# glmanhtu/vit-ed

Measured on AMD Instinct MI355X. Metric: patch-pairs/sec fwd+bwd, div2k_erosion7_4bin_patch8_64 ViT-ED, higher is better.
Workload: dtype bf16

## Files before the change

### vit-ed_amd/csrc/context_fold.hip

```cpp
#include "common.h"

#define CF_MAX_BLOCKS 16

struct FoldArgs {
    const float* w[CF_MAX_BLOCKS];
    const float* bias[CF_MAX_BLOCKS];
    const float* gamma[CF_MAX_BLOCKS];
    const float* beta[CF_MAX_BLOCKS];
    bf16* w_out;
    bf16* wt_out;
    float* bias_out;
    int count, N, K;
};

__global__ void __launch_bounds__(256) fold_context_kernel(const FoldArgs a) {
    const int lane = threadIdx.x & 63;
    const int row = blockIdx.x * 4 + (threadIdx.x >> 6);
    if (row >= a.count * a.N) return;
    const int l = row / a.N, n = row - l * a.N;
    const float* __restrict__ w = a.w[l] + (int64_t)n * a.K;
    const float* __restrict__ g = a.gamma[l];
    const float* __restrict__ be = a.beta[l];
    const int64_t ldt = (int64_t)a.count * a.N;
    float dot = 0.f;
    for (int k = lane; k < a.K; k += 64) {
        const float wv = w[k];
        const bf16 f = (bf16)(wv * g[k]);
        a.w_out[(int64_t)row * a.K + k] = f;
        a.wt_out[(int64_t)k * ldt + row] = f;
        dot = fmaf(wv, be[k], dot);
    }
    dot = wave_sum(dot);
    if (lane == 0) a.bias_out[row] = dot + (a.bias[l] ? a.bias[l][n] : 0.f);
}

extern "C" int vited_fold_context_weights(int count, const float* const* w, const float* const* bias, const float* const* gamma,
                                          const float* const* beta, int64_t N, int64_t K, void* w_out, void* wt_out, float* bias_out,
                                          void* stream) {
    if (count < 1 || count > CF_MAX_BLOCKS || !w || !bias || !gamma || !beta || !w_out || !wt_out || !bias_out || N <= 0 || K <= 0)
        return VITED_ERR_BAD_ARG;
    FoldArgs a = {};
    for (int i = 0; i < count; ++i) {
        if (!w[i] || !gamma[i] || !beta[i]) return VITED_ERR_BAD_ARG;
        a.w[i] = w[i]; a.bias[i] = bias[i]; a.gamma[i] = gamma[i]; a.beta[i] = beta[i];
    }
    a.w_out = (bf16*)w_out; a.wt_out = (bf16*)wt_out; a.bias_out = bias_out;
    a.count = count; a.N = (int)N; a.K = (int)K;
    hipLaunchKernelGGL(fold_context_kernel, dim3((unsigned)ceil_div64((int64_t)count * N, 4)), dim3(256), 0, (hipStream_t)stream, a);
    return vited_check_launch();
}

struct UnfoldArgs {
    const float* w[CF_MAX_BLOCKS];
    const float* gamma[CF_MAX_BLOCKS];
    const float* beta[CF_MAX_BLOCKS];
    float* dw[CF_MAX_BLOCKS];
    float* dbias[CF_MAX_BLOCKS];
    float* dgamma[CF_MAX_BLOCKS];
    float* dbeta[CF_MAX_BLOCKS];
    const float* dwf;
    const float* dbf;
    int count, N, K, accumulate;
};

#define UF_GROUPS 16
__global__ void __launch_bounds__(64 * UF_GROUPS) unfold_context_kernel(const UnfoldArgs a) {
    __shared__ float red[2][UF_GROUPS][64];
    const int l = blockIdx.y, kx = threadIdx.x & 63, ng = threadIdx.x >> 6;
    const int k = blockIdx.x * 64 + kx;
    const bool ok = k < a.K;
    const float* __restrict__ w = a.w[l];
    const float* __restrict__ dwf = a.dwf + (int64_t)l * a.N * a.K;
    const float* __restrict__ dbf = a.dbf + (int64_t)l * a.N;
    float* __restrict__ dw = a.dw[l];
    const float g = ok ? a.gamma[l][k] : 0.f, be = ok ? a.beta[l][k] : 0.f;
    float sg = 0.f, sb = 0.f;
#pragma unroll 4
    for (int n = ng; n < a.N; n += UF_GROUPS) {
        if (ok) {
            const int64_t o = (int64_t)n * a.K + k;
            const float d = dwf[o], wv = w[o], dbn = dbf[n];
            sg = fmaf(d, wv, sg);
            sb = fmaf(dbn, wv, sb);
            const float v = fmaf(d, g, dbn * be);
            dw[o] = a.accumulate ? dw[o] + v : v;
        }
    }
    red[0][ng][kx] = sg;
    red[1][ng][kx] = sb;
    __syncthreads();
    if (ng == 0 && ok) {
        float tg = 0.f, tb = 0.f;
#pragma unroll
        for (int w = 0; w < UF_GROUPS; ++w) {
            tg += red[0][w][kx];
            tb += red[1][w][kx];
        }
        a.dgamma[l][k] = a.accumulate ? a.dgamma[l][k] + tg : tg;
        a.dbeta[l][k] = a.accumulate ? a.dbeta[l][k] + tb : tb;
    }
    if (blockIdx.x == 0 && a.dbias[l]) {
        for (int n = threadIdx.x; n < a.N; n += 64 * UF_GROUPS) a.dbias[l][n] = a.accumulate ? a.dbias[l][n] + dbf[n] : dbf[n];
    }
}

extern "C" int vited_unfold_context_grads(int count, const float* dwf, const float* dbf, const float* const* w, const float* const* gamma,
                                          const float* const* beta, float* const* dw, float* const* dbias, float* const* dgamma, float* const* dbeta, int64_t N,
                                          int64_t K, int accumulate, void* stream) {
    if (count < 1 || count > CF_MAX_BLOCKS || !dwf || !dbf || !w || !gamma || !beta || !dw || !dbias || !dgamma || !dbeta || N <= 0 || K <= 0)
        return VITED_ERR_BAD_ARG;
    UnfoldArgs a = {};
    for (int i = 0; i < count; ++i) {
        if (!w[i] || !gamma[i] || !beta[i] || !dw[i] || !dgamma[i] || !dbeta[i]) return VITED_ERR_BAD_ARG;
        a.w[i] = w[i]; a.gamma[i] = gamma[i]; a.beta[i] = beta[i]; a.dw[i] = dw[i]; a.dbias[i] = dbias[i]; a.dgamma[i] = dgamma[i]; a.dbeta[i] = dbeta[i];
    }
    a.dwf = dwf; a.dbf = dbf; a.count = count; a.N = (int)N; a.K = (int)K; a.accumulate = accumulate;
    hipLaunchKernelGGL(unfold_context_kernel, dim3((unsigned)ceil_div64(K, 64), (unsigned)count), dim3(64 * UF_GROUPS), 0, (hipStream_t)stream, a);
    return vited_check_launch();
}
```

### vit-ed_amd/csrc/elementwise.hip

```cpp
#include "common.h"

template <typename S, typename D>
__global__ void cast_kernel(const S* __restrict__ src, D* __restrict__ dst, int64_t n) {
    int64_t i = ((int64_t)blockIdx.x * blockDim.x + threadIdx.x) * 4;
    const int64_t stride = (int64_t)gridDim.x * blockDim.x * 4;
    for (; i + 3 < n; i += stride) {
        S a = src[i], b = src[i + 1], c = src[i + 2], d = src[i + 3];
        dst[i] = from_f32<D>(to_f32(a));
        dst[i + 1] = from_f32<D>(to_f32(b));
        dst[i + 2] = from_f32<D>(to_f32(c));
        dst[i + 3] = from_f32<D>(to_f32(d));
    }
    for (; i < n; ++i) dst[i] = from_f32<D>(to_f32(src[i]));
}

extern "C" int vited_cast(const void* src, int src_dtype, void* dst, int dst_dtype, int64_t n, void* stream) {
    if (!src || !dst || n < 0) return VITED_ERR_BAD_ARG;
    if (n == 0) return VITED_OK;
    hipStream_t s = (hipStream_t)stream;
    const int threads = 256;
    int64_t blocks = ceil_div64(n, threads * 4);
    if (blocks > 4096) blocks = 4096;
    if (src_dtype == VITED_F32 && dst_dtype == VITED_BF16)
        hipLaunchKernelGGL((cast_kernel<float, bf16>), dim3(blocks), dim3(threads), 0, s, (const float*)src, (bf16*)dst, n);
    else if (src_dtype == VITED_BF16 && dst_dtype == VITED_F32)
        hipLaunchKernelGGL((cast_kernel<bf16, float>), dim3(blocks), dim3(threads), 0, s, (const bf16*)src, (float*)dst, n);
    else if (src_dtype == VITED_F32 && dst_dtype == VITED_F32)
        hipLaunchKernelGGL((cast_kernel<float, float>), dim3(blocks), dim3(threads), 0, s, (const float*)src, (float*)dst, n);
    else if (src_dtype == VITED_BF16 && dst_dtype == VITED_BF16)
        hipLaunchKernelGGL((cast_kernel<bf16, bf16>), dim3(blocks), dim3(threads), 0, s, (const bf16*)src, (bf16*)dst, n);
    else
        return VITED_ERR_UNSUPPORTED;
    return vited_check_launch();
}

template <typename D>
__global__ void __launch_bounds__(256)
scale_rows_cast_kernel(const float* __restrict__ src, int64_t src_ld, const float* __restrict__ scale, D* __restrict__ dst, int64_t dst_ld,
                       int64_t rows, int dim) {
    const int hl = threadIdx.x & 31;
    const int64_t half = ((int64_t)blockIdx.x * blockDim.x + threadIdx.x) >> 5;
    const int64_t nhalf = ((int64_t)gridDim.x * blockDim.x) >> 5;
    for (int64_t r = half; r < rows; r += nhalf) {
        const float sc = scale[r];
        for (int c = hl * 4; c < dim; c += 128) {
            const f32x4 v = *(const f32x4*)(src + r * src_ld + c);
            if constexpr (sizeof(D) == 2) {
                *(bf16x4*)((bf16*)dst + r * dst_ld + c) = bf16x4{(bf16)(sc * v[0]), (bf16)(sc * v[1]), (bf16)(sc * v[2]), (bf16)(sc * v[3])};
            } else {
                *(f32x4*)((float*)dst + r * dst_ld + c) = f32x4{sc * v[0], sc * v[1], sc * v[2], sc * v[3]};
            }
        }
    }
}

extern "C" int vited_scale_rows_cast(const float* src, int64_t src_ld, const float* row_scale, void* dst, int dst_dtype, int64_t dst_ld,
                                     int64_t rows, int64_t dim, void* stream) {
    if (!src || !row_scale || !dst || rows <= 0 || dim <= 0 || src_ld < dim || dst_ld < dim) return VITED_ERR_BAD_ARG;
    if (dim % 4 || src_ld % 4 || dst_ld % 4 || dim > (1 << 20)) return VITED_ERR_UNSUPPORTED;
    if (((uintptr_t)src & 15) || ((uintptr_t)dst & (dst_dtype == VITED_F32 ? 15 : 7))) return VITED_ERR_BAD_ARG;
    int64_t blocks = ceil_div64(rows, 8);
    if (blocks > 2048) blocks = 2048;
    hipStream_t s = (hipStream_t)stream;
    if (dst_dtype == VITED_BF16)
        hipLaunchKernelGGL((scale_rows_cast_kernel<bf16>), dim3(blocks), dim3(256), 0, s, src, src_ld, row_scale, (bf16*)dst, dst_ld, rows, (int)dim);
    else if (dst_dtype == VITED_F32)
        hipLaunchKernelGGL((scale_rows_cast_kernel<float>), dim3(blocks), dim3(256), 0, s, src, src_ld, row_scale, (float*)dst, dst_ld, rows, (int)dim);
    else
        return VITED_ERR_UNSUPPORTED;
    return vited_check_launch();
}

template <typename D>
__global__ void cast_transpose_kernel(const float* __restrict__ src, D* __restrict__ dst, int64_t rows, int64_t cols) {
    __shared__ float tile[32][33];
    const int64_t c0 = (int64_t)blockIdx.x * 32, r0 = (int64_t)blockIdx.y * 32;
    const int tx = threadIdx.x & 31, ty = threadIdx.x >> 5;
    for (int j = ty; j < 32; j += 8) {
        int64_t r = r0 + j, c = c0 + tx;
        tile[j][tx] = (r < rows && c < cols) ? src[r * cols + c] : 0.f;
    }
    __syncthreads();
    for (int j = ty; j < 32; j += 8) {
        int64_t c = c0 + j, r = r0 + tx;
        if (c < cols && r < rows) dst[c * rows + r] = from_f32<D>(tile[tx][j]);
    }
}

extern "C" int vited_cast_transpose(const float* src, void* dst, int dst_dtype, int64_t rows, int64_t cols, void* stream) {
    if (!src || !dst || rows <= 0 || cols <= 0) return VITED_ERR_BAD_ARG;
    dim3 grid((unsigned)ceil_div64(cols, 32), (unsigned)ceil_div64(rows, 32));
    hipStream_t s = (hipStream_t)stream;
    if (dst_dtype == VITED_BF16)
        hipLaunchKernelGGL((cast_transpose_kernel<bf16>), grid, dim3(256), 0, s, src, (bf16*)dst, rows, cols);
    else if (dst_dtype == VITED_F32)
        hipLaunchKernelGGL((cast_transpose_kernel<float>), grid, dim3(256), 0, s, src, (float*)dst, rows, cols);
    else
        return VITED_ERR_UNSUPPORTED;
    return vited_check_launch();
}

#define WS_DESC_WORDS 6
__global__ void __launch_bounds__(256)
cast_weights_kernel(const int64_t* __restrict__ desc, int count) {
    __shared__ bf16 tile[64][66];
    const int64_t blk = blockIdx.x;
    int lo = 0, hi = count - 1;
    while (lo < hi) {
        const int mid = (lo + hi + 1) >> 1;
        if (desc[(int64_t)mid * WS_DESC_WORDS + 5] <= blk) lo = mid; else hi = mid - 1;
    }
    const int64_t* d = desc + (int64_t)lo * WS_DESC_WORDS;
    const float* __restrict__ src = (const float*)d[0];
    bf16* __restrict__ dst = (bf16*)d[1];
    bf16* __restrict__ dst_t = (bf16*)d[2];
    const int64_t rows = d[3], cols = d[4];
    const int64_t t = blk - d[5], tiles_c = (cols + 63) >> 6;
    const int64_t r0 = (t / tiles_c) << 6, c0 = (t % tiles_c) << 6;
    const int tx = threadIdx.x & 15, ty = threadIdx.x >> 4;
    const bool vec = (cols & 3) == 0;
#pragma unroll
    for (int j = 0; j < 4; ++j) {
        const int lr = ty + 16 * j;
        const int64_t r = r0 + lr, c = c0 + tx * 4;
        float v[4] = {0.f, 0.f, 0.f, 0.f};
        if (r < rows) {
            if (vec && c + 3 < cols) {
                const f32x4 q = *(const f32x4*)(src + r * cols + c);
                v[0] = q[0]; v[1] = q[1]; v[2] = q[2]; v[3] = q[3];
            } else {
#pragma unroll
                for (int e = 0; e < 4; ++e) if (c + e < cols) v[e] = src[r * cols + c + e];
            }
        }
        bf16 b[4];
#pragma unroll
        for (int e = 0; e < 4; ++e) { b[e] = (bf16)v[e]; tile[lr][tx * 4 + e] = b[e]; }
        if (dst && r < rows) {
            if (vec && c + 3 < cols) *(bf16x4*)(dst + r * cols + c) = bf16x4{b[0], b[1], b[2], b[3]};
            else {
#pragma unroll
                for (int e = 0; e < 4; ++e) if (c + e < cols) dst[r * cols + c + e] = b[e];
            }
        }
    }
    if (!dst_t) return;
    __syncthreads();
    const bool vec_t = (rows & 3) == 0;
#pragma unroll
    for (int j = 0; j < 4; ++j) {
        const int lc = ty + 16 * j;
        const int64_t c = c0 + lc, r = r0 + tx * 4;
        if (c >= cols) continue;
        bf16 b[4];
#pragma unroll
        for (int e = 0; e < 4; ++e) b[e] = tile[tx * 4 + e][lc];
        if (vec_t && r + 3 < rows) *(bf16x4*)(dst_t + c * rows + r) = bf16x4{b[0], b[1], b[2], b[3]};
        else {
#pragma unroll
            for (int e = 0; e < 4; ++e) if (r + e < rows) dst_t[c * rows + r + e] = b[e];
        }
    }
}

extern "C" int vited_cast_weights(const int64_t* desc, int count, int64_t total_tiles, void* stream) {
    if (!desc || count <= 0 || total_tiles <= 0 || total_tiles > 0x7fffffff) return VITED_ERR_BAD_ARG;
    hipLaunchKernelGGL(cast_weights_kernel, dim3((unsigned)total_tiles), dim3(256), 0, (hipStream_t)stream, desc, count);
    return vited_check_launch();
}

template <typename D>
__global__ void patchify_kernel(const float* __restrict__ img, int64_t img_bs, const int64_t* __restrict__ bidx,
                                D* __restrict__ out, int chans, int S, int p) {
    const int G = S / p;
    const int64_t b = blockIdx.y;
    const int py = blockIdx.x;
    const int64_t src_b = bidx ? bidx[b] : b;
    const float* base = img + src_b * img_bs;
    const int Kp = chans * p * p;
    const int total = chans * p * S;
    D* obase = out + (b * G * G + (int64_t)py * G) * Kp;
    for (int e = threadIdx.x; e < total; e += blockDim.x) {
        const int x = e % S;
        const int ci = e / S;
        const int i = ci % p, c = ci / p;
        const float v = base[((int64_t)c * S + (py * p + i)) * S + x];
        const int px = x / p, j = x - px * p;
        obase[(int64_t)px * Kp + (c * p + i) * p + j] = from_f32<D>(v);
    }
}

extern "C" int vited_patchify(const float* img, int64_t img_bs, const int64_t* batch_index, void* out, int out_dtype,
                              int64_t batch, int chans, int img_size, int patch, void* stream) {
    if (!img || !out || batch <= 0 || chans <= 0 || img_size <= 0 || patch <= 0 || img_size % patch) return VITED_ERR_BAD_ARG;
    dim3 grid(img_size / patch, (unsigned)batch);
    hipStream_t s = (hipStream_t)stream;
    if (out_dtype == VITED_BF16)
        hipLaunchKernelGGL((patchify_kernel<bf16>), grid, dim3(256), 0, s, img, img_bs, batch_index, (bf16*)out, chans, img_size, patch);
    else if (out_dtype == VITED_F32)
        hipLaunchKernelGGL((patchify_kernel<float>), grid, dim3(256), 0, s, img, img_bs, batch_index, (float*)out, chans, img_size, patch);
    else
        return VITED_ERR_UNSUPPORTED;
    return vited_check_launch();
}

struct U8Norm { float scale[4], shift[4]; };

template <typename D>
__global__ void patchify_u8_kernel(const uint8_t* __restrict__ img, int64_t img_bs, const int64_t* __restrict__ bidx,
                                   D* __restrict__ out, int chans, int S, int p, U8Norm nrm) {
    const int G = S / p;
    const int64_t b = blockIdx.y;
    const int py = blockIdx.x;
    const int64_t src_b = bidx ? bidx[b] : b;
    const uint8_t* base = img + src_b * img_bs;
    const int Kp = chans * p * p;
    const int total = chans * p * S;
    D* obase = out + (b * G * G + (int64_t)py * G) * Kp;
    for (int e = threadIdx.x; e < total; e += blockDim.x) {
        const int x = e % S;
        const int ci = e / S;
        const int i = ci % p, c = ci / p;
        const float v = fmaf((float)base[((int64_t)c * S + (py * p + i)) * S + x], nrm.scale[c], nrm.shift[c]);
        const int px = x / p, j = x - px * p;
        obase[(int64_t)px * Kp + (c * p + i) * p + j] = from_f32<D>(v);
    }
}

extern "C" int vited_patchify_u8(const uint8_t* img, int64_t img_bs, const int64_t* batch_index, void* out, int out_dtype,
                                 int64_t batch, int chans, int img_size, int patch, const float* mean, const float* std,
                                 void* stream) {
    if (!img || !out || !mean || !std || batch <= 0 || chans <= 0 || chans > 4 || img_size <= 0 || patch <= 0 || img_size % patch)
        return VITED_ERR_BAD_ARG;
    U8Norm nrm = {};
    for (int c = 0; c < chans; ++c) {
        if (!(std[c] > 0.f)) return VITED_ERR_BAD_ARG;
        nrm.scale[c] = 1.0f / (255.0f * std[c]);
        nrm.shift[c] = -mean[c] / std[c];
    }
    dim3 grid(img_size / patch, (unsigned)batch);
    hipStream_t s = (hipStream_t)stream;
    if (out_dtype == VITED_BF16)
        hipLaunchKernelGGL((patchify_u8_kernel<bf16>), grid, dim3(256), 0, s, img, img_bs, batch_index, (bf16*)out, chans, img_size, patch, nrm);
    else if (out_dtype == VITED_F32)
        hipLaunchKernelGGL((patchify_u8_kernel<float>), grid, dim3(256), 0, s, img, img_bs, batch_index, (float*)out, chans, img_size, patch, nrm);
    else
        return VITED_ERR_UNSUPPORTED;
    return vited_check_launch();
}

struct ResampleTaps {
    int x0, n;
    int k0, k1;
};

__device__ __forceinline__ ResampleTaps resample_taps(int xx, int in_size, int out_size) {
    constexpr int PRECISION_BITS = 32 - 8 - 2;
    const double scale = (double)in_size / (double)out_size;
    const double center = (xx + 0.5) * scale;
    int xmin = (int)(center - 1.0 + 0.5);
    xmin = xmin < 0 ? 0 : xmin;
    int xmax = (int)(center + 1.0 + 0.5);
    xmax = (xmax < in_size ? xmax : in_size) - xmin;
    double w0 = 1.0 - fabs((double)xmin - center + 0.5), w1 = xmax > 1 ? 1.0 - fabs((double)xmin + 1.0 - center + 0.5) : 0.0;
    w0 = w0 < 0.0 ? 0.0 : w0;
    w1 = w1 < 0.0 ? 0.0 : w1;
    const double ww = w0 + w1;
    ResampleTaps t;
    t.x0 = xmin;
    t.n = xmax > 1 ? 2 : 1;
    t.k0 = (int)(0.5 + (w0 / ww) * (double)(1 << PRECISION_BITS));
    t.k1 = (int)(0.5 + (w1 / ww) * (double)(1 << PRECISION_BITS));
    return t;
}

__device__ __forceinline__ int resample_px(int p0, int p1, const ResampleTaps& t) {
    constexpr int PRECISION_BITS = 32 - 8 - 2;
    int acc = (1 << (PRECISION_BITS - 1)) + p0 * t.k0 + (t.n > 1 ? p1 * t.k1 : 0);
    acc >>= PRECISION_BITS;
    return acc < 0 ? 0 : (acc > 255 ? 255 : acc);
}

__global__ void __launch_bounds__(256)
crop_pairs_u8_kernel(const uint8_t* __restrict__ src, int64_t src_bs, const int* __restrict__ cells, const int* __restrict__ erode,
                     uint8_t* __restrict__ out, int chans, int S) {
    const int64_t b = blockIdx.z;
    const int img = blockIdx.y / chans, c = blockIdx.y % chans;
    int cell = cells[b * 2 + img], e = erode[b];
    cell = cell < 0 ? 0 : (cell > 5 ? 5 : cell);
    e = e < 1 ? 1 : (e > S ? S : e);
    const int off = (int)rint((S - e) / 2.0);
    const int r0 = (cell / 3) * S + off, c0 = (cell % 3) * S + off;
    const uint8_t* base = src + b * src_bs + ((int64_t)c * 2 * S + r0) * (3 * S) + c0;
    uint8_t* o = out + (((b * 2 + img) * chans + c) * (int64_t)S) * S;
    for (int i = blockIdx.x * blockDim.x + threadIdx.x; i < S * S; i += gridDim.x * blockDim.x) {
        const int y = i / S, x = i - y * S;
        const ResampleTaps tx = resample_taps(x, e, S), ty = resample_taps(y, e, S);
        const uint8_t* ra = base + (int64_t)ty.x0 * (3 * S) + tx.x0;
        const int h0 = resample_px(ra[0], tx.n > 1 ? ra[1] : 0, tx);
        int h1 = 0;
        if (ty.n > 1) {
            const uint8_t* rb = ra + 3 * S;
            h1 = resample_px(rb[0], tx.n > 1 ? rb[1] : 0, tx);
        }
        o[i] = (uint8_t)resample_px(h0, h1, ty);
    }
}

extern "C" int vited_crop_pairs_u8(const uint8_t* src, int64_t src_bs, const int* cells, const int* erode, uint8_t* out, int64_t batch,
                                   int chans, int img_size, void* stream) {
    if (!src || !cells || !erode || !out || batch <= 0 || chans <= 0 || img_size <= 0 || batch > 65535) return VITED_ERR_BAD_ARG;
    if (src_bs < (int64_t)chans * 6 * img_size * img_size) return VITED_ERR_BAD_ARG;
    const int per = img_size * img_size;
    dim3 grid((unsigned)((per + 1023) / 1024 < 8 ? (per + 1023) / 1024 : 8), (unsigned)(2 * chans), (unsigned)batch);
    hipLaunchKernelGGL(crop_pairs_u8_kernel, grid, dim3(256), 0, (hipStream_t)stream, src, src_bs, cells, erode, out, chans, img_size);
    return vited_check_launch();
}

template <typename D>
__global__ void slice_rows_cast_kernel(const float* __restrict__ in, D* __restrict__ out, int64_t in_rows,
                                       int64_t row_offset, int64_t rows, int64_t dim, int64_t total) {
    int64_t i = (int64_t)blockIdx.x * blockDim.x + threadIdx.x;
    const int64_t stride = (int64_t)gridDim.x * blockDim.x;
    const int64_t per_b = rows * dim;
    for (; i < total; i += stride) {
        const int64_t b = i / per_b, rem = i - b * per_b;
        out[i] = from_f32<D>(in[(b * in_rows + row_offset) * dim + rem]);
    }
}

extern "C" int vited_slice_rows_cast(const float* in, void* out, int out_dtype, int64_t batch, int64_t in_rows,
                                     int64_t row_offset, int64_t rows, int64_t dim, void* stream) {
    if (!in || !out || batch <= 0 || rows <= 0 || dim <= 0 || row_offset < 0 || row_offset + rows > in_rows) return VITED_ERR_BAD_ARG;
    const int64_t total = batch * rows * dim;
    int64_t blocks = ceil_div64(total, 256);
    if (blocks > 8192) blocks = 8192;
    hipStream_t s = (hipStream_t)stream;
    if (out_dtype == VITED_BF16)
        hipLaunchKernelGGL((slice_rows_cast_kernel<bf16>), dim3(blocks), dim3(256), 0, s, in, (bf16*)out, in_rows, row_offset, rows, dim, total);
    else if (out_dtype == VITED_F32)
        hipLaunchKernelGGL((slice_rows_cast_kernel<float>), dim3(blocks), dim3(256), 0, s, in, (float*)out, in_rows, row_offset, rows, dim, total);
    else
        return VITED_ERR_UNSUPPORTED;
    return vited_check_launch();
}

__global__ void write_cls_row_kernel(float* __restrict__ x, const float* __restrict__ cls, const float* __restrict__ pos,
                                     int64_t batch, int64_t rows_per_batch, int64_t dim) {
    int64_t i = (int64_t)blockIdx.x * blockDim.x + threadIdx.x;
    const int64_t total = batch * dim;
    if (i >= total) return;
    const int64_t b = i / dim, d = i - b * dim;
    x[b * rows_per_batch * dim + d] = cls[d] + pos[d];
}

extern "C" int vited_write_cls_row(float* x, const float* cls, const float* pos, int64_t batch, int64_t rows_per_batch,
                                   int64_t dim, void* stream) {
    if (!x || !cls || !pos || batch <= 0 || rows_per_batch <= 0 || dim <= 0) return VITED_ERR_BAD_ARG;
    const int64_t total = batch * dim;
    hipLaunchKernelGGL(write_cls_row_kernel, dim3((unsigned)ceil_div64(total, 256)), dim3(256), 0, (hipStream_t)stream,
                       x, cls, pos, batch, rows_per_batch, dim);
    return vited_check_launch();
}

template <typename S_>
__global__ void sum_rows_kernel(const S_* __restrict__ in, int64_t in_ld, float* __restrict__ out, int64_t batch,
                                int64_t width, int64_t rows_per_split) {
    const int64_t r = (int64_t)blockIdx.x * blockDim.x + threadIdx.x;
    if (r >= width) return;
    const int64_t b0 = (int64_t)blockIdx.y * rows_per_split;
    int64_t b1 = b0 + rows_per_split;
    if (b1 > batch) b1 = batch;
    float acc0 = 0.f, acc1 = 0.f, acc2 = 0.f, acc3 = 0.f;
    int64_t b = b0;
    for (; b + 3 < b1; b += 4) {
        acc0 += to_f32(in[b * in_ld + r]);
        acc1 += to_f32(in[(b + 1) * in_ld + r]);
        acc2 += to_f32(in[(b + 2) * in_ld + r]);
        acc3 += to_f32(in[(b + 3) * in_ld + r]);
    }
    for (; b < b1; ++b) acc0 += to_f32(in[b * in_ld + r]);
    out[(int64_t)blockIdx.y * width + r] = (acc0 + acc1) + (acc2 + acc3);
}

static inline int64_t sum_rows_splits(int64_t batch, int64_t width) {
    const int64_t col_blocks = ceil_div64(width, 256);
    int64_t s = ceil_div64(1024, col_blocks);
    const int64_t max_s = ceil_div64(batch, 16);
    if (s > max_s) s = max_s;
    if (s < 1) s = 1;
    return s;
}

extern "C" int64_t vited_sum_rows_workspace_bytes(int64_t batch, int64_t width) {
    return sum_rows_splits(batch, width) * width * (int64_t)sizeof(float);
// ... 165 lines not shown
```

### vit-ed_amd/csrc/patch_keep.hip

```cpp
#include "common.h"
#include "patch_keep.h"

__global__ void __launch_bounds__(256)
keep_from_keys_kernel(const float* __restrict__ keys, int* __restrict__ keep, int L, int K) {
    __shared__ float row[PK_MAX_KEYS];
    const int64_t b = blockIdx.x;
    const float* src = keys + b * L;
    for (int i = threadIdx.x; i < L; i += blockDim.x) row[i] = src[i];
    __syncthreads();
    for (int i = threadIdx.x; i < L; i += blockDim.x) {
        const int rank = pk_rank(row, L, i);
        if (rank < K) keep[b * K + rank] = i;
    }
}

extern "C" int vited_keep_from_keys(const float* keys, int32_t* keep, int64_t batch, int L, int K, void* stream) {
    if (!keys || !keep || batch <= 0 || batch > 0x7fffffff || L <= 0 || K <= 0 || K > L) return VITED_ERR_BAD_ARG;
    if (((uintptr_t)keys | (uintptr_t)keep) % 4) return VITED_ERR_BAD_ARG;
    if (L > PK_MAX_KEYS) return VITED_ERR_UNSUPPORTED;
    hipLaunchKernelGGL(keep_from_keys_kernel, dim3((unsigned)batch), dim3(256), 0, (hipStream_t)stream, keys, keep, L, K);
    return vited_check_launch();
}

struct PkNorm { float scale[4], shift[4]; };

template <typename S, typename D>
__global__ void __launch_bounds__(256)
patchify_kept_kernel(const S* __restrict__ img, int64_t img_bs, const int64_t* __restrict__ bidx, const int* __restrict__ keep, int K,
                     int lead, D* __restrict__ out, int chans, int img_size, int p, PkNorm nrm) {
    const int G = img_size / p, R = pk_rows(K, lead);
    const int64_t b = blockIdx.x;
    const int r = blockIdx.y;
    const int patch = pk_patch(keep + b * K, lead, r, G * G);
    const int py = patch / G, px = patch - py * G;
    const int64_t src_b = bidx ? bidx[b] : b;
    const S* base = img + src_b * img_bs + (int64_t)(py * p) * img_size + px * p;
    const int Kp = chans * p * p;
    D* o = out + (b * R + r) * (int64_t)Kp;
    for (int e = threadIdx.x; e < Kp; e += blockDim.x) {
        const int j = e % p, ci = e / p;
        const int i = ci % p, c = ci / p;
        const S raw = base[((int64_t)c * img_size + i) * img_size + j];
        float v;
        if constexpr (sizeof(S) == 1) v = fmaf((float)raw, nrm.scale[c], nrm.shift[c]);
        else v = raw;
        o[e] = from_f32<D>(v);
    }
}

static int patchify_kept_args(const void* img, const int32_t* keep, int K, int lead, const void* out, int64_t batch, int chans,
                              int img_size, int patch) {
    if (!img || !keep || !out || batch <= 0 || batch > 0x7fffffff || chans <= 0 || img_size <= 0 || patch <= 0 || img_size % patch)
        return VITED_ERR_BAD_ARG;
    const int64_t n = (int64_t)(img_size / patch) * (img_size / patch);
    if ((lead != 0 && lead != 1) || K <= 0 || (int64_t)K + lead > n || (uintptr_t)keep % 4) return VITED_ERR_BAD_ARG;
    if (pk_rows(K, lead) > 65535) return VITED_ERR_UNSUPPORTED;
    return VITED_OK;
}

extern "C" int vited_patchify_kept(const float* img, int64_t img_bs, const int64_t* batch_index, const int32_t* keep, int K, int lead,
                                   void* out, int out_dtype, int64_t batch, int chans, int img_size, int patch, void* stream) {
    if (int err = patchify_kept_args(img, keep, K, lead, out, batch, chans, img_size, patch)) return err;
    if ((uintptr_t)img % 4) return VITED_ERR_BAD_ARG;
    dim3 grid((unsigned)batch, (unsigned)pk_rows(K, lead));
    hipStream_t s = (hipStream_t)stream;
    const PkNorm none = {};
    if (out_dtype == VITED_BF16)
        hipLaunchKernelGGL((patchify_kept_kernel<float, bf16>), grid, dim3(256), 0, s, img, img_bs, batch_index, keep, K, lead, (bf16*)out,
                           chans, img_size, patch, none);
    else if (out_dtype == VITED_F32)
        hipLaunchKernelGGL((patchify_kept_kernel<float, float>), grid, dim3(256), 0, s, img, img_bs, batch_index, keep, K, lead, (float*)out,
                           chans, img_size, patch, none);
    else
        return VITED_ERR_UNSUPPORTED;
    return vited_check_launch();
}

extern "C" int vited_patchify_kept_u8(const uint8_t* img, int64_t img_bs, const int64_t* batch_index, const int32_t* keep, int K, int lead,
                                      void* out, int out_dtype, int64_t batch, int chans, int img_size, int patch, const float* mean,
                                      const float* std, void* stream) {
    if (int err = patchify_kept_args(img, keep, K, lead, out, batch, chans, img_size, patch)) return err;
    if (!mean || !std || chans > 4) return VITED_ERR_BAD_ARG;
    PkNorm nrm = {};
    for (int c = 0; c < chans; ++c) {
        if (!(std[c] > 0.f)) return VITED_ERR_BAD_ARG;
        nrm.scale[c] = 1.0f / (255.0f * std[c]);
        nrm.shift[c] = -mean[c] / std[c];
    }
    dim3 grid((unsigned)batch, (unsigned)pk_rows(K, lead));
    hipStream_t s = (hipStream_t)stream;
    if (out_dtype == VITED_BF16)
        hipLaunchKernelGGL((patchify_kept_kernel<uint8_t, bf16>), grid, dim3(256), 0, s, img, img_bs, batch_index, keep, K, lead, (bf16*)out,
                           chans, img_size, patch, nrm);
    else if (out_dtype == VITED_F32)
        hipLaunchKernelGGL((patchify_kept_kernel<uint8_t, float>), grid, dim3(256), 0, s, img, img_bs, batch_index, keep, K, lead,
                           (float*)out, chans, img_size, patch, nrm);
    else
        return VITED_ERR_UNSUPPORTED;
    return vited_check_launch();
}

__global__ void __launch_bounds__(256)
tokens_kept_kernel(const float* __restrict__ tok, const float* __restrict__ pos, const float* __restrict__ cls, const int* __restrict__ keep,
                   int K, int lead, float* __restrict__ x, int64_t total, int n_patches, int dim4) {
    const int R = pk_rows(K, lead), first = cls ? 1 : 0, rows = R + first;
    const int64_t stride = (int64_t)gridDim.x * blockDim.x;
    for (int64_t i = (int64_t)blockIdx.x * blockDim.x + threadIdx.x; i < total; i += stride) {
        const int64_t row = i / dim4;
        const int c = (int)(i - row * dim4) * 4;
        const int64_t b = row / rows;
        const int t = (int)(row - b * rows);
        f32x4 v;
        if (t < first) {
            v = *(const f32x4*)(cls + c) + *(const f32x4*)(pos + c);
        } else {
            const int r = t - first;
            const int patch = pk_patch(keep + b * K, lead, r, n_patches);
            v = *(const f32x4*)(tok + (b * R + r) * (int64_t)(dim4 * 4) + c) + *(const f32x4*)(pos + (int64_t)(1 + patch) * (dim4 * 4) + c);
        }
        *(f32x4*)(x + row * (int64_t)(dim4 * 4) + c) = v;
    }
}

extern "C" int vited_tokens_kept(const float* tok, const float* pos, const float* cls, const int32_t* keep, int K, int lead, float* x,
                                 int64_t batch, int n_patches, int dim, void* stream) {
    if (!tok || !pos || !keep || !x || batch <= 0 || n_patches <= 0 || dim <= 0 || dim % 4) return VITED_ERR_BAD_ARG;
    if ((lead != 0 && lead != 1) || K <= 0 || (int64_t)K + lead > n_patches || (uintptr_t)keep % 4) return VITED_ERR_BAD_ARG;
    if (((uintptr_t)tok | (uintptr_t)pos | (uintptr_t)cls | (uintptr_t)x) % 16) return VITED_ERR_BAD_ARG;
    const int64_t total = batch * (pk_rows(K, lead) + (cls ? 1 : 0)) * (dim / 4);
    int64_t blocks = ceil_div64(total, 256);
    if (blocks > 8192) blocks = 8192;
    hipLaunchKernelGGL(tokens_kept_kernel, dim3((unsigned)blocks), dim3(256), 0, (hipStream_t)stream, tok, pos, cls, keep, K, lead, x, total,
                       n_patches, dim / 4);
    return vited_check_launch();
}

__global__ void __launch_bounds__(256)
keep_inverse_kernel(const int* __restrict__ keep, int K, int lead, int* __restrict__ inv, int n_patches) {
    const int64_t b = blockIdx.x;
    int* mine = inv + b * n_patches;
    pk_inverse_clear(mine, n_patches, threadIdx.x, blockDim.x);
    __syncthreads();
    pk_inverse_fill(mine, keep + b * K, K, lead, n_patches, threadIdx.x, blockDim.x);
}

extern "C" int vited_keep_inverse(const int32_t* keep, int K, int lead, int32_t* inv, int64_t batch, int n_patches, void* stream) {
    if (!keep || !inv || batch <= 0 || batch > 0x7fffffff || n_patches <= 0) return VITED_ERR_BAD_ARG;
    if ((lead != 0 && lead != 1) || K <= 0 || (int64_t)K + lead > n_patches || ((uintptr_t)keep | (uintptr_t)inv) % 4) return VITED_ERR_BAD_ARG;
    hipLaunchKernelGGL(keep_inverse_kernel, dim3((unsigned)batch), dim3(256), 0, (hipStream_t)stream, keep, K, lead, inv, n_patches);
    return vited_check_launch();
}

__global__ void __launch_bounds__(256)
tokens_kept_bwd_kernel(const float* __restrict__ dx, const int* __restrict__ inv, float* __restrict__ dpos, float* __restrict__ dcls,
                       int64_t batch, int rows, int first, int n_patches, int dim4) {
    const int64_t i = (int64_t)blockIdx.x * blockDim.x + threadIdx.x;
    if (i >= (int64_t)(n_patches + 1) * dim4) return;
    const int q = (int)(i / dim4), c = (int)(i - (int64_t)q * dim4) * 4;
    const int dim = dim4 * 4, R = rows - first;
    f32x4 acc = {0.f, 0.f, 0.f, 0.f};
    if (q == 0) {
        if (first)
            for (int64_t b = 0; b < batch; ++b) acc += *(const f32x4*)(dx + b * rows * (int64_t)dim + c);
        if (dcls) *(f32x4*)(dcls + c) = acc;
    } else {
        const int* col = inv + (q - 1);
        int64_t b = 0;
        for (; b + 4 <= batch; b += 4) {
            int r[4];
#pragma unroll
            for (int u = 0; u < 4; ++u) r[u] = col[(b + u) * n_patches];
            f32x4 v[4];
#pragma unroll
            for (int u = 0; u < 4; ++u) {
                const bool kept = r[u] >= 0 && r[u] < R;
                v[u] = kept ? *(const f32x4*)(dx + ((b + u) * rows + first + (kept ? r[u] : 0)) * (int64_t)dim + c) : f32x4{0.f, 0.f, 0.f, 0.f};
            }
#pragma unroll
            for (int u = 0; u < 4; ++u)
                if (r[u] >= 0 && r[u] < R) acc += v[u];
        }
        for (; b < batch; ++b) {
            const int r = col[b * n_patches];
            if (r >= 0 && r < R) acc += *(const f32x4*)(dx + (b * rows + first + r) * (int64_t)dim + c);
        }
    }
    *(f32x4*)(dpos + (int64_t)q * dim + c) = acc;
}

extern "C" int vited_tokens_kept_bwd(const float* dx, const int32_t* inv, float* dpos, float* dcls, int64_t batch, int rows, int with_cls,
                                     int n_patches, int dim, void* stream) {
    if (!dx || !inv || !dpos || batch <= 0 || n_patches <= 0 || dim <= 0 || dim % 4 || (with_cls != 0 && with_cls != 1)) return VITED_ERR_BAD_ARG;
    if (rows <= with_cls || rows - with_cls > n_patches || (!with_cls && dcls)) return VITED_ERR_BAD_ARG;
    if (((uintptr_t)dx | (uintptr_t)dpos | (uintptr_t)dcls) % 16 || (uintptr_t)inv % 4) return VITED_ERR_BAD_ARG;
    const int64_t total = (int64_t)(n_patches + 1) * (dim / 4);
    hipLaunchKernelGGL(tokens_kept_bwd_kernel, dim3((unsigned)ceil_div64(total, 256)), dim3(256), 0, (hipStream_t)stream, dx, inv, dpos,
                       dcls, batch, rows, with_cls, n_patches, dim / 4);
    return vited_check_launch();
}
```

Baseline: 43860.

## Tile context fold transpose, deepen unfold loads, vectorise patchify row runs

The context-weight fold kernel now processes 32 rows per block and stages results in shared memory, so the transposed bf16 output is written as coalesced 4-wide vectors instead of strided scalar stores. The unfold gradient kernel is templated on column width and accumulate mode, batches many loads ahead of use for memory-level parallelism, and picks a narrower width when the grid would be small. The patchify and kept-patchify paths gain kernels where each thread moves one contiguous patch row with vector loads and stores, falling back to the old kernels when alignment fails. A profiling helper script is added. Register pressure from the deeper unrolling and extra template instances are the main risks.

Measured after the change: 43890, median of 3. No clear change (+0.1%).

```diff
diff --git a/profiles/step_kernels.py b/profiles/step_kernels.py
--- /dev/null
+++ b/profiles/step_kernels.py
@@ -0,0 +1,53 @@
+#!/usr/bin/env python3
+import collections
+import csv
+import glob
+import os
+import statistics
+import sys
+
+
+def main():
+    args = [a for a in sys.argv[1:] if not a.startswith('--')]
+    src, dst = args[0], args[1]
+    window = None
+    if '--window' in sys.argv:
+        window = int(sys.argv[sys.argv.index('--window') + 1])
+    trace = max(glob.glob(os.path.join(src, '**', '*_kernel_trace.csv'), recursive=True), key=os.path.getmtime)
+    rows = []
+    for r in csv.DictReader(open(trace)):
+        rows.append((int(r['Start_Timestamp']), int(r['End_Timestamp']), r['Kernel_Name']))
+    rows.sort()
+    os.makedirs(dst, exist_ok=True)
+
+    per = collections.defaultdict(list)
+    for s, e, n in rows:
+        per[n].append(e - s)
+    with open(os.path.join(dst, 'kernel_stats.csv'), 'w') as f:
+        f.write('Name,Calls,TotalDurationNs,AverageNs,MedianNs\n')
+        for n, d in sorted(per.items(), key=lambda kv: -sum(kv[1]))[:60]:
+            f.write(f'"{n[:110]}",{len(d)},{sum(d)},{sum(d) // len(d)},{int(statistics.median(d))}\n')
+
+    ends = [i for i, (_, _, n) in enumerate(rows) if 'optim_update_kernel' in n or 'adamw_update_kernel' in n]
+    first_u8 = next((i for i, (_, _, n) in enumerate(rows) if 'patchify_u8' in n or 'patchify_run_kernelIh' in n
+                     or 'patchify_run_kernel<unsigned char' in n), len(rows))
+    wins = [(ends[k - 1] + 1, ends[k] + 1) for k in range(1, len(ends))]
+    for k, (a, b) in enumerate(wins):
+        print(f'window {k}: {b - a} kernels, wall {(rows[b - 1][1] - rows[a][0]) / 1e6:.3f} ms, '
+              f'busy {sum(e - s for s, e, _ in rows[a:b]) / 1e6:.3f} ms')
+    if window is None:
+        window = max(k for k, (a, b) in enumerate(wins) if b <= first_u8)
+    a, b = wins[window]
+    print(f'chosen window {window}')
+    step = collections.defaultdict(list)
+    for s, e, n in rows[a:b]:
+        step[n].append(e - s)
+    with open(os.path.join(dst, 'step_kernels.csv'), 'w') as f:
+        f.write('Name,Launches,TotalUs,AverageUs\n')
+        for n, d in sorted(step.items(), key=lambda kv: -sum(kv[1])):
+            f.write(f'"{n[:110]}",{len(d)},{sum(d) / 1e3:.2f},{sum(d) / len(d) / 1e3:.2f}\n')
+    print(f'step: {b - a} kernels, wall {(rows[b - 1][1] - rows[a][0]) / 1e6:.3f} ms, busy {sum(e - s for s, e, _ in rows[a:b]) / 1e6:.3f} ms')
+
+
+if __name__ == '__main__':
+    main()
diff --git a/vit-ed_amd/csrc/context_fold.hip b/vit-ed_amd/csrc/context_fold.hip
--- a/vit-ed_amd/csrc/context_fold.hip
+++ b/vit-ed_amd/csrc/context_fold.hip
@@ -13,25 +13,72 @@
     int count, N, K;
 };
 
+#define FC_ROWS 32
+#define FC_PER_WAVE (FC_ROWS / 4)
 __global__ void __launch_bounds__(256) fold_context_kernel(const FoldArgs a) {
-    const int lane = threadIdx.x & 63;
-    const int row = blockIdx.x * 4 + (threadIdx.x >> 6);
-    if (row >= a.count * a.N) return;
-    const int l = row / a.N, n = row - l * a.N;
-    const float* __restrict__ w = a.w[l] + (int64_t)n * a.K;
-    const float* __restrict__ g = a.gamma[l];
-    const float* __restrict__ be = a.beta[l];
-    const int64_t ldt = (int64_t)a.count * a.N;
-    float dot = 0.f;
-    for (int k = lane; k < a.K; k += 64) {
-        const float wv = w[k];
-        const bf16 f = (bf16)(wv * g[k]);
-        a.w_out[(int64_t)row * a.K + k] = f;
-        a.wt_out[(int64_t)k * ldt + row] = f;
-        dot = fmaf(wv, be[k], dot);
+    __shared__ bf16 tile[64][FC_ROWS + 4];
+    const int lane = threadIdx.x & 63, wave = threadIdx.x >> 6;
+    const int rows = a.count * a.N;
+    const int row0 = blockIdx.x * FC_ROWS;
+    const int64_t ldt = rows;
+    const bool vec_t = (ldt & 3) == 0 && ((uintptr_t)a.wt_out & 7) == 0;
+    const float* w[FC_PER_WAVE];
+    const float* g[FC_PER_WAVE];
+    const float* be[FC_PER_WAVE];
+    float dot[FC_PER_WAVE];
+#pragma unroll
+    for (int j = 0; j < FC_PER_WAVE; ++j) {
+        const int row = row0 + wave * FC_PER_WAVE + j;
+        const int l = row < rows ? row / a.N : 0, n = row < rows ? row - l * a.N : 0;
+        w[j] = a.w[l] + (int64_t)n * a.K;
+        g[j] = a.gamma[l];
+        be[j] = a.beta[l];
+        dot[j] = 0.f;
     }
-    dot = wave_sum(dot);
-    if (lane == 0) a.bias_out[row] = dot + (a.bias[l] ? a.bias[l][n] : 0.f);
+    for (int k0 = 0; k0 < a.K; k0 += 64) {
+        const int k = k0 + lane;
+        float wv[FC_PER_WAVE], gv[FC_PER_WAVE], bv[FC_PER_WAVE];
+#pragma unroll
+        for (int j = 0; j < FC_PER_WAVE; ++j) {
+            const bool ok = k < a.K && row0 + wave * FC_PER_WAVE + j < rows;
+            wv[j] = ok ? w[j][k] : 0.f;
+            gv[j] = ok ? g[j][k] : 0.f;
+            bv[j] = ok ? be[j][k] : 0.f;
+        }
+#pragma unroll
+        for (int j = 0; j < FC_PER_WAVE; ++j) {
+            const int row = row0 + wave * FC_PER_WAVE + j;
+            const bf16 f = (bf16)(wv[j] * gv[j]);
+            tile[lane][wave * FC_PER_WAVE + j] = f;
+            if (k < a.K && row < rows) {
+                a.w_out[(int64_t)row * a.K + k] = f;
+                dot[j] = fmaf(wv[j], bv[j], dot[j]);
+            }
+        }
+        __syncthreads();
+#pragma unroll
+        for (int q = threadIdx.x; q < 64 * (FC_ROWS / 4); q += 256) {
+            const int r4 = (q % (FC_ROWS / 4)) * 4, kk = q / (FC_ROWS / 4);
+            const int row = row0 + r4;
+            if (k0 + kk >= a.K || row >= rows) continue;
+            bf16* dst = a.wt_out + (int64_t)(k0 + kk) * ldt + row;
+            if (vec_t && row + 3 < rows) *(bf16x4*)dst = *(const bf16x4*)&tile[kk][r4];
+            else {
+                for (int e = 0; e < 4; ++e)
+                    if (row + e < rows) dst[e] = tile[kk][r4 + e];
+            }
+        }
+        __syncthreads();
+    }
+#pragma unroll
+    for (int j = 0; j < FC_PER_WAVE; ++j) {
+        const int row = row0 + wave * FC_PER_WAVE + j;
+        const float d = wave_sum(dot[j]);
+        if (lane == 0 && row < rows) {
+            const int l = row / a.N, n = row - l * a.N;
+            a.bias_out[row] = d + (a.bias[l] ? a.bias[l][n] : 0.f);
+        }
+    }
 }
 
 extern "C" int vited_fold_context_weights(int count, const float* const* w, const float* const* bias, const float* const* gamma,
@@ -46,7 +93,7 @@
     }
     a.w_out = (bf16*)w_out; a.wt_out = (bf16*)wt_out; a.bias_out = bias_out;
     a.count = count; a.N = (int)N; a.K = (int)K;
-    hipLaunchKernelGGL(fold_context_kernel, dim3((unsigned)ceil_div64((int64_t)count * N, 4)), dim3(256), 0, (hipStream_t)stream, a);
+    hipLaunchKernelGGL(fold_context_kernel, dim3((unsigned)ceil_div64((int64_t)count * N, FC_ROWS)), dim3(256), 0, (hipStream_t)stream, a);
     return vited_check_launch();
 }
 
@@ -64,10 +111,17 @@
 };
 
 #define UF_GROUPS 16
-__global__ void __launch_bounds__(64 * UF_GROUPS) unfold_context_kernel(const UnfoldArgs a) {
-    __shared__ float red[2][UF_GROUPS][64];
-    const int l = blockIdx.y, kx = threadIdx.x & 63, ng = threadIdx.x >> 6;
-    const int k = blockIdx.x * 64 + kx;
+#ifndef UF_MIN_BLOCKS
+#define UF_MIN_BLOCKS 96
+#endif
+#ifndef UF_DEPTH
+#define UF_DEPTH 24
+#endif
+template <int COLS, bool ACC>
+__global__ void __launch_bounds__(COLS * UF_GROUPS) unfold_context_kernel(const UnfoldArgs a) {
+    __shared__ float red[2][UF_GROUPS][COLS];
+    const int l = blockIdx.y, kx = threadIdx.x % COLS, ng = threadIdx.x / COLS;
+    const int k = blockIdx.x * COLS + kx;
     const bool ok = k < a.K;
     const float* __restrict__ w = a.w[l];
     const float* __restrict__ dwf = a.dwf + (int64_t)l * a.N * a.K;
@@ -75,15 +129,28 @@
     float* __restrict__ dw = a.dw[l];
     const float g = ok ? a.gamma[l][k] : 0.f, be = ok ? a.beta[l][k] : 0.f;
     float sg = 0.f, sb = 0.f;
-#pragma unroll 4
-    for (int n = ng; n < a.N; n += UF_GROUPS) {
-        if (ok) {
+    constexpr int DEPTH = COLS == 64 ? UF_DEPTH / 3 : COLS == 32 ? UF_DEPTH * 2 / 3 : UF_DEPTH;
+    for (int n0 = ng; n0 < a.N; n0 += UF_GROUPS * DEPTH) {
+        float d[DEPTH], wv[DEPTH], dbn[DEPTH], old[DEPTH];
+#pragma unroll
+        for (int u = 0; u < DEPTH; ++u) {
+            const int n = n0 + u * UF_GROUPS;
+            const bool in = ok && n < a.N;
             const int64_t o = (int64_t)n * a.K + k;
-            const float d = dwf[o], wv = w[o], dbn = dbf[n];
-            sg = fmaf(d, wv, sg);
-            sb = fmaf(dbn, wv, sb);
-            const float v = fmaf(d, g, dbn * be);
-            dw[o] = a.accumulate ? dw[o] + v : v;
+            d[u] = in ? dwf[o] : 0.f;
+            wv[u] = in ? w[o] : 0.f;
+            dbn[u] = in ? dbf[n] : 0.f;
+            old[u] = (ACC && in) ? dw[o] : 0.f;
+        }
+#pragma unroll
+        for (int u = 0; u < DEPTH; ++u) {
+            const int n = n0 + u * UF_GROUPS;
+            if (ok && n < a.N) {
+                sg = fmaf(d[u], wv[u], sg);
+                sb = fmaf(dbn[u], wv[u], sb);
+                const float v = fmaf(d[u], g, dbn[u] * be);
+                dw[(int64_t)n * a.K + k] = ACC ? old[u] + v : v;
+            }
         }
     }
     red[0][ng][kx] = sg;
@@ -96,12 +163,19 @@
             tg += red[0][w][kx];
             tb += red[1][w][kx];
         }
-        a.dgamma[l][k] = a.accumulate ? a.dgamma[l][k] + tg : tg;
-        a.dbeta[l][k] = a.accumulate ? a.dbeta[l][k] + tb : tb;
+        a.dgamma[l][k] = ACC ? a.dgamma[l][k] + tg : tg;
+        a.dbeta[l][k] = ACC ? a.dbeta[l][k] + tb : tb;
     }
     if (blockIdx.x == 0 && a.dbias[l]) {
-        for (int n = threadIdx.x; n < a.N; n += 64 * UF_GROUPS) a.dbias[l][n] = a.accumulate ? a.dbias[l][n] + dbf[n] : dbf[n];
+        for (int n = threadIdx.x; n < a.N; n += COLS * UF_GROUPS) a.dbias[l][n] = ACC ? a.dbias[l][n] + dbf[n] : dbf[n];
     }
+}
+
+template <int COLS>
+static void unfold_launch(const UnfoldArgs& a, hipStream_t s) {
+    const dim3 grid((unsigned)ceil_div64(a.K, COLS), (unsigned)a.count), block(COLS * UF_GROUPS);
+    if (a.accumulate) hipLaunchKernelGGL((unfold_context_kernel<COLS, true>), grid, block, 0, s, a);
+    else hipLaunchKernelGGL((unfold_context_kernel<COLS, false>), grid, block, 0, s, a);
 }
 
 extern "C" int vited_unfold_context_grads(int count, const float* dwf, const float* dbf, const float* const* w, const float* const* gamma,
@@ -115,6 +189,9 @@
         a.w[i] = w[i]; a.gamma[i] = gamma[i]; a.beta[i] = beta[i]; a.dw[i] = dw[i]; a.dbias[i] = dbias[i]; a.dgamma[i] = dgamma[i]; a.dbeta[i] = dbeta[i];
     }
     a.dwf = dwf; a.dbf = dbf; a.count = count; a.N = (int)N; a.K = (int)K; a.accumulate = accumulate;
-    hipLaunchKernelGGL(unfold_context_kernel, dim3((unsigned)ceil_div64(K, 64), (unsigned)count), dim3(64 * UF_GROUPS), 0, (hipStream_t)stream, a);
+    hipStream_t s = (hipStream_t)stream;
+    if (ceil_div64(K, 64) * count >= UF_MIN_BLOCKS) unfold_launch<64>(a, s);
+    else if (ceil_div64(K, 32) * count >= UF_MIN_BLOCKS) unfold_launch<32>(a, s);
+    else unfold_launch<16>(a, s);
     return vited_check_launch();
 }
diff --git a/vit-ed_amd/csrc/elementwise.hip b/vit-ed_amd/csrc/elementwise.hip
--- a/vit-ed_amd/csrc/elementwise.hip
+++ b/vit-ed_amd/csrc/elementwise.hip
@@ -1,4 +1,5 @@
 #include "common.h"
+#include "patch_run.h"
 
 template <typename S, typename D>
 __global__ void cast_kernel(const S* __restrict__ src, D* __restrict__ dst, int64_t n) {
@@ -167,6 +168,59 @@
     if (!desc || count <= 0 || total_tiles <= 0 || total_tiles > 0x7fffffff) return VITED_ERR_BAD_ARG;
     hipLaunchKernelGGL(cast_weights_kernel, dim3((unsigned)total_tiles), dim3(256), 0, (hipStream_t)stream, desc, count);
     return vited_check_launch();
+}
+
+template <typename S, typename D, int P>
+__global__ void __launch_bounds__(256)
+patchify_run_kernel(const S* __restrict__ img, int64_t img_bs, const int64_t* __restrict__ bidx, D* __restrict__ out, int chans,
+                    int img_size, unsigned G, int g_shift, unsigned total, PatchNorm nrm) {
+    const unsigned t = blockIdx.x * 256u + threadIdx.x;
+    if (t >= total) return;
+    unsigned px, u, py;
+    int64_t b;
+    if (g_shift >= 0) {
+        px = t & (G - 1), u = t >> g_shift;
+    } else {
+        px = t % G, u = t / G;
+    }
+    const unsigned i = u % P, strip = u / P;
+    if (g_shift >= 0) {
+        py = strip & (G - 1), b = strip >> g_shift;
+    } else {
+        py = strip % G, b = strip / G;
+    }
+    const int64_t src_b = bidx ? bidx[b] : b;
+    const int64_t plane = (int64_t)img_size * img_size;
+    const S* __restrict__ src = img + src_b * img_bs + (int64_t)(py * P + i) * img_size + px * P;
+    D* __restrict__ dst = out + ((int64_t)strip * G + px) * ((int64_t)chans * P * P) + i * P;
+    if (chans == 3) {
+#pragma unroll
+        for (int c = 0; c < 3; ++c) patch_run_move<S, D, P>(src + c * plane, dst + c * P * P, nrm.scale[c], nrm.shift[c]);
+    } else {
+        for (int c = 0; c < chans; ++c) patch_run_move<S, D, P>(src + c * plane, dst + c * P * P, nrm.scale[c & 3], nrm.shift[c & 3]);
+    }
+}
+
+template <typename S, typename D>
+static bool patchify_runs(const S* img, int64_t img_bs, const int64_t* bidx, D* out, int64_t batch, int chans, int img_size, int p,
+                          const PatchNorm& nrm, hipStream_t s) {
+    if (!patch_runs_vectorisable(img, img_bs, sizeof(S), out, sizeof(D), p)) return false;
+    const int64_t total = batch * img_size * (img_size / p);
+    if (total > 0x7fffffff) return false;
+    const dim3 grid((unsigned)ceil_div64(total, 256));
+    const unsigned G = img_size / p;
+    int g_shift = -1;
+    if ((G & (G - 1)) == 0)
+        for (g_shift = 0; (1u << g_shift) < G; ++g_shift) {}
+#define PATCHIFY_RUN_CASE(P) \
+    case P: hipLaunchKernelGGL((patchify_run_kernel<S, D, P>), grid, dim3(256), 0, s, img, img_bs, bidx, out, chans, img_size, G, g_shift, \
+                               (unsigned)total, nrm); break;
+    switch (p) {
+        PATCHIFY_RUN_CASE(2) PATCHIFY_RUN_CASE(4) PATCHIFY_RUN_CASE(8) PATCHIFY_RUN_CASE(16) PATCHIFY_RUN_CASE(32)
+        default: return false;
+    }
+#undef PATCHIFY_RUN_CASE
+    return true;
 }
 
 template <typename D>
@@ -195,7 +249,10 @@
     if (!img || !out || batch <= 0 || chans <= 0 || img_size <= 0 || patch <= 0 || img_size % patch) return VITED_ERR_BAD_ARG;
     dim3 grid(img_size / patch, (unsigned)batch);
     hipStream_t s = (hipStream_t)stream;
-    if (out_dtype == VITED_BF16)
+    const PatchNorm none = {};
+    if (out_dtype == VITED_BF16 && patchify_runs(img, img_bs, batch_index, (bf16*)out, batch, chans, img_size, patch, none, s)) {
+    } else if (out_dtype == VITED_F32 && patchify_runs(img, img_bs, batch_index, (float*)out, batch, chans, img_size, patch, none, s)) {
+    } else if (out_dtype == VITED_BF16)
         hipLaunchKernelGGL((patchify_kernel<bf16>), grid, dim3(256), 0, s, img, img_bs, batch_index, (bf16*)out, chans, img_size, patch);
     else if (out_dtype == VITED_F32)
         hipLaunchKernelGGL((patchify_kernel<float>), grid, dim3(256), 0, s, img, img_bs, batch_index, (float*)out, chans, img_size, patch);
@@ -204,7 +261,7 @@
     return vited_check_launch();
 }
 
-struct U8Norm { float scale[4], shift[4]; };
+typedef PatchNorm U8Norm;
 
 template <typename D>
 __global__ void patchify_u8_kernel(const uint8_t* __restrict__ img, int64_t img_bs, const int64_t* __restrict__ bidx,
@@ -240,7 +297,9 @@
     }
     dim3 grid(img_size / patch, (unsigned)batch);
     hipStream_t s = (hipStream_t)stream;
-    if (out_dtype == VITED_BF16)
+    if (out_dtype == VITED_BF16 && patchify_runs(img, img_bs, batch_index, (bf16*)out, batch, chans, img_size, patch, nrm, s)) {
+    } else if (out_dtype == VITED_F32 && patchify_runs(img, img_bs, batch_index, (float*)out, batch, chans, img_size, patch, nrm, s)) {
+    } else if (out_dtype == VITED_BF16)
         hipLaunchKernelGGL((patchify_u8_kernel<bf16>), grid, dim3(256), 0, s, img, img_bs, batch_index, (bf16*)out, chans, img_size, patch, nrm);
     else if (out_dtype == VITED_F32)
         hipLaunchKernelGGL((patchify_u8_kernel<float>), grid, dim3(256), 0, s, img, img_bs, batch_index, (float*)out, chans, img_size, patch, nrm);
diff --git a/vit-ed_amd/csrc/patch_keep.hip b/vit-ed_amd/csrc/patch_keep.hip
--- a/vit-ed_amd/csrc/patch_keep.hip
+++ b/vit-ed_amd/csrc/patch_keep.hip
@@ -1,5 +1,6 @@
 #include "common.h"
 #include "patch_keep.h"
+#include "patch_run.h"
 
 __global__ void __launch_bounds__(256)
 keep_from_keys_kernel(const float* __restrict__ keys, int* __restrict__ keep, int L, int K) {
@@ -22,7 +23,7 @@
     return vited_check_launch();
 }
 
-struct PkNorm { float scale[4], shift[4]; };
+typedef PatchNorm PkNorm;
 
 template <typename S, typename D>
 __global__ void __launch_bounds__(256)
@@ -48,6 +49,48 @@
     }
 }
 
+template <typename S, typename D, int P>
+__global__ void __launch_bounds__(256)
+patchify_kept_run_kernel(const S* __restrict__ img, int64_t img_bs, const int64_t* __restrict__ bidx, const int* __restrict__ keep, int K,
+                         int lead, D* __restrict__ out, int chans, int img_size, unsigned total, PatchNorm nrm) {
+    const unsigned t = blockIdx.x * 256u + threadIdx.x;
+    if (t >= total) return;
+    const unsigned G = img_size / P, R = pk_rows(K, lead);
+    const unsigned i = t % P, row = t / P;
+    const unsigned r = row % R;
+    const int64_t b = row / R;
+    const unsigned patch = pk_patch(keep + b * K, lead, (int)r, (int)(G * G));
+    const unsigned py = patch / G, px = patch - py * G;
+    const int64_t src_b = bidx ? bidx[b] : b;
+    const int64_t plane = (int64_t)img_size * img_size;
+    const S* __restrict__ src = img + src_b * img_bs + (int64_t)(py * P + i) * img_size + px * P;
+    D* __restrict__ dst = out + (int64_t)row * ((int64_t)chans * P * P) + i * P;
+    if (chans == 3) {
+#pragma unroll
+        for (int c = 0; c < 3; ++c) patch_run_move<S, D, P>(src + c * plane, dst + c * P * P, nrm.scale[c], nrm.shift[c]);
+    } else {
+        for (int c = 0; c < chans; ++c) patch_run_move<S, D, P>(src + c * plane, dst + c * P * P, nrm.scale[c & 3], nrm.shift[c & 3]);
+    }
+}
+
+template <typename S, typename D>
+static bool patchify_kept_runs(const S* img, int64_t img_bs, const int64_t* bidx, const int* keep, int K, int lead, D* out, int64_t batch,
+                               int chans, int img_size, int p, const PatchNorm& nrm, hipStream_t s) {
+    if (!patch_runs_vectorisable(img, img_bs, sizeof(S), out, sizeof(D), p)) return false;
+    const int64_t total = batch * pk_rows(K, lead) * p;
+    if (total > 0x7fffffff) return false;
+    const dim3 grid((unsigned)ceil_div64(total, 256));
+#define PATCHIFY_KEPT_CASE(P) \
+    case P: hipLaunchKernelGGL((patchify_kept_run_kernel<S, D, P>), grid, dim3(256), 0, s, img, img_bs, bidx, keep, K, lead, out, chans, \
+                               img_size, (unsigned)total, nrm); break;
+    switch (p) {
+        PATCHIFY_KEPT_CASE(2) PATCHIFY_KEPT_CASE(4) PATCHIFY_KEPT_CASE(8) PATCHIFY_KEPT_CASE(16) PATCHIFY_KEPT_CASE(32)
+        default: return false;
+    }
+#undef PATCHIFY_KEPT_CASE
+    return true;
+}
+
 static int patchify_kept_args(const void* img, const int32_t* keep, int K, int lead, const void* out, int64_t batch, int chans,
                               int img_size, int patch) {
     if (!img || !keep || !out || batch <= 0 || batch > 0x7fffffff || chans <= 0 || img_size <= 0 || patch <= 0 || img_size % patch)
@@ -65,7 +108,10 @@
     dim3 grid((unsigned)batch, (unsigned)pk_rows(K, lead));
     hipStream_t s = (hipStream_t)stream;
     const PkNorm none = {};
-    if (out_dtype == VITED_BF16)
+    if (out_dtype == VITED_BF16 && patchify_kept_runs(img, img_bs, batch_index, keep, K, lead, (bf16*)out, batch, chans, img_size, patch, none, s)) {
+    } else if (out_dtype == VITED_F32 &&
+               patchify_kept_runs(img, img_bs, batch_index, keep, K, lead, (float*)out, batch, chans, img_size, patch, none, s)) {
+    } else if (out_dtype == VITED_BF16)
         hipLaunchKernelGGL((patchify_kept_kernel<float, bf16>), grid, dim3(256), 0, s, img, img_bs, batch_index, keep, K, lead, (bf16*)out,
                            chans, img_size, patch, none);
     else if (out_dtype == VITED_F32)
@@ -89,7 +135,10 @@
     }
     dim3 grid((unsigned)batch, (unsigned)pk_rows(K, lead));
     hipStream_t s = (hipStream_t)stream;
-    if (out_dtype == VITED_BF16)
+    if (out_dtype == VITED_BF16 && patchify_kept_runs(img, img_bs, batch_index, keep, K, lead, (bf16*)out, batch, chans, img_size, patch, nrm, s)) {
+    } else if (out_dtype == VITED_F32 &&
+               patchify_kept_runs(img, img_bs, batch_index, keep, K, lead, (float*)out, batch, chans, img_size, patch, nrm, s)) {
+    } else if (out_dtype == VITED_BF16)
         hipLaunchKernelGGL((patchify_kept_kernel<uint8_t, bf16>), grid, dim3(256), 0, s, img, img_bs, batch_index, keep, K, lead, (bf16*)out,
                            chans, img_size, patch, nrm);
     else if (out_dtype == VITED_F32)
diff --git a/vit-ed_amd/csrc/patch_run.h b/vit-ed_amd/csrc/patch_run.h
--- /dev/null
+++ b/vit-ed_amd/csrc/patch_run.h
@@ -0,0 +1,30 @@
+#pragma once
+#include "common.h"
+
+template <typename T, int N> struct alignas(sizeof(T) * N > 16 ? 16 : sizeof(T) * N) PatchRun { T v[N]; };
+
+struct PatchNorm { float scale[4], shift[4]; };
+
+static inline int patch_run_width(int p) { return (p == 2 || p == 4 || p == 8 || p == 16 || p == 32) ? p : 0; }
+
+static inline bool patch_runs_vectorisable(const void* img, int64_t img_bs, size_t in_size, const void* out, size_t out_size, int p) {
+    if (!patch_run_width(p)) return false;
+    const size_t in_run = (size_t)p * in_size, out_run = (size_t)p * out_size;
+    if (in_run % 4 || out_run % 4) return false;
+    const size_t in_al = in_run > 16 ? 16 : in_run, out_al = out_run > 16 ? 16 : out_run;
+    return (uintptr_t)img % in_al == 0 && ((uint64_t)img_bs * in_size) % in_al == 0 && (uintptr_t)out % out_al == 0;
+}
+
+template <typename S, typename D, int P>
+__device__ __forceinline__ void patch_run_move(const S* __restrict__ src, D* __restrict__ dst, float scale, float shift) {
+    const PatchRun<S, P> in = *(const PatchRun<S, P>*)src;
+    PatchRun<D, P> o;
+#pragma unroll
+    for (int j = 0; j < P; ++j) {
+        float v;
+        if constexpr (sizeof(S) == 1) v = fmaf((float)in.v[j], scale, shift);
+        else v = in.v[j];
+        o.v[j] = from_f32<D>(v);
+    }
+    *(PatchRun<D, P>*)dst = o;
+}
```
